# ericdegroot/gr-ldpc_ece535a

Measured on AMD Instinct MI355X. Metric: decoded info Mbit/s @ 50 BP iters, batch=4096; achieved HBM GB/s vs peak, higher is better.
Workload: dtype f64

## Files before the change

### gr-ldpc_ece535a_amd/csrc/ldpc_capi_create.hip

```cpp
#include <stdio.h>

#include <exception>

#include "ldpc_ctx.hpp"
#include "ldpc_layout.hpp"
#include "ldpc_qc.hpp"

using namespace ldpc::capi;
using ldpc::ColRec;
using ldpc::EdgeColRec;
using ldpc::EdgeRowRec;
using ldpc::kNone;

namespace ldpc {
namespace capi {

int set_err(ldpc_ctx *ctx, int code, const std::string &msg) {
  if (!ctx) return set_create_error(code, msg);
  ctx->err = msg;
  return code;
}

int hip_err(ldpc_ctx *ctx, hipError_t e, const char *what) {
  return set_err(ctx, LDPC_EDEVICE, std::string(what) + ": " + hipGetErrorString(e));
// ... 52 lines not shown
        row_edges[j].push_back(e);
        col_edges[i].push_back(e);
      }
  code.E = (int)erow.size();
  code.dc_max = 0;
  code.dv_max = 0;
  for (auto &r : row_edges) code.dc_max = std::max(code.dc_max, (int)r.size());
  code.dc_min = code.dc_max;
  for (auto &r : row_edges) code.dc_min = std::min(code.dc_min, (int)r.size());
  for (auto &c : col_edges) code.dv_max = std::max(code.dv_max, (int)c.size());
  if (code.E == 0) return set_err(ctx, LDPC_EINVAL, "H has no ones");
  if (N > ldpc::kNMax || M > ldpc::kMMax || code.E > 64 * ldpc::kSlotsMax ||
      code.dc_max > ldpc::kDcMax || code.dv_max > ldpc::kDvMax) {
    char buf[256];
    snprintf(buf, sizeof buf,
             "code shape outside the small-code kernel (M=%d N=%d E=%d dc_max=%d dv_max=%d; "
             "limits M,N<=%d E<=%d dc<=%d dv<=%d)",
             M, N, code.E, code.dc_max, code.dv_max, ldpc::kNMax, 64 * ldpc::kSlotsMax,
             ldpc::kDcMax, ldpc::kDvMax);
    return set_err(ctx, LDPC_EUNSUPPORTED, buf);
  }
  ctx->slots = (code.E + 63) / 64;
  ctx->nw = N <= 64 ? 1 : 4;
  ctx->rs = (M + 63) / 64;
  const int slots = ctx->slots, nw = ctx->nw;
  code.K = N - M;
  code.KB = (code.K + 7) / 8;

  const ldpc::KernelShape shape = ldpc::kernel_shape(nw, slots, code.dc_max, code.dv_max);
  const ldpc::EdgeLayout lay = ldpc::plan_layout(M, N, erow, ecol, slots, nw, shape.dcn, shape.dvn,
                                                 shape.cols, search);
  const std::vector<int> &cell = lay.slot, &pos = lay.pos;
  if (cell_out) *cell_out = cell;
  int *model = ctx->small.layout_model;
  model[0] = lay.searched ? 1 : 0;
  model[1] = lay.model_cc;
  model[2] = lay.model_ec;
  model[3] = lay.plain_cc;
  model[4] = lay.plain_ec;
  uint64_t *dpos = ctx->small.dpos;
  dpos[0] = dpos[1] = 0;
  for (int g = 0; g < 2 * slots; ++g) dpos[g / 8] |= (uint64_t)(lay.dpos[g] & 31) << (8 * (g % 8));

  erecs.assign((size_t)64 * slots, EdgeRowRec{});
  crecs.assign((size_t)64 * slots, EdgeColRec{});
  for (auto &r : erecs) {
    std::fill(std::begin(r.rn), std::end(r.rn), kNone);
    r.col = kNone;
  }
  for (auto &r : crecs) {
    std::fill(std::begin(r.cn), std::end(r.cn), kNone);
    r.col = kNone;
  }
  for (int e = 0; e < code.E; ++e) {
    EdgeRowRec &er = erecs[cell[e]];
    EdgeColRec &ec = crecs[cell[e]];
    er.col = ec.col = (uint16_t)pos[ecol[e]];
    int k = 0;
    for (int n : row_edges[erow[e]])
      if (n != e) er.rn[k++] = (uint16_t)cell[n];
    k = 0;
    for (int n : col_edges[ecol[e]])
      if (n != e) ec.cn[k++] = (uint16_t)cell[n];
  }
  cols.assign((size_t)64 * nw, ColRec{});
  for (auto &c : cols) {
    std::fill(std::begin(c.e), std::end(c.e), kNone);
    std::fill(std::begin(c.r), std::end(c.r), kNone);
  }
  lane_col.assign((size_t)64 * nw, kNone);
  col_lane.assign((size_t)N, 0);
  for (int i = 0; i < N; ++i) {
    lane_col[pos[i]] = (uint16_t)i;
    col_lane[i] = (uint8_t)pos[i];
    for (size_t k = 0; k < col_edges[i].size(); ++k) {
      cols[pos[i]].e[k] = (uint16_t)cell[col_edges[i][k]];
      cols[pos[i]].r[k] = (uint16_t)erow[col_edges[i][k]];
    }
  }
  rowmask.assign((size_t)M * nw, 0);
  for (int j = 0; j < M; ++j)
    for (int i = 0; i < N; ++i)
      if (H[(size_t)j * N + i]) rowmask[(size_t)j * nw + pos[i] / 64] |= 1ull << (pos[i] % 64);
  return LDPC_OK;
}

int build_graph(ldpc_ctx *ctx, std::vector<int32_t> &cp, std::vector<int32_t> &ce,
                std::vector<int32_t> &cr) {
  ldpc_ctx::Code &code = ctx->code;
  const int M = code.M, N = code.N;
  code.E = code.rp[M];
  if (code.E == 0) return set_err(ctx, LDPC_EINVAL, "H has no ones");
  cp.assign((size_t)N + 1, 0);
  for (int e = 0; e < code.E; ++e) cp[code.ci[e] + 1]++;
  code.dc_max = 0;
  code.dv_max = 0;
  for (int i = 0; i < N; ++i) code.dv_max = std::max(code.dv_max, cp[i + 1]);
  for (int j = 0; j < M; ++j) code.dc_max = std::max(code.dc_max, code.rp[j + 1] - code.rp[j]);
  for (int i = 0; i < N; ++i) cp[i + 1] += cp[i];
  ce.assign((size_t)code.E, 0);
  cr.assign((size_t)code.E, 0);
  std::vector<int32_t> fill(cp.begin(), cp.end() - 1);
  for (int j = 0; j < M; ++j)
    for (int32_t e = code.rp[j]; e < code.rp[j + 1]; ++e) {
      const int32_t k = fill[code.ci[e]]++;
      ce[k] = e;
      cr[k] = j;
    }
  if (code.dc_max > ldpc::kGraphDcMax || code.dv_max > ldpc::kGraphDvMax) {
    char buf[160];
    snprintf(buf, sizeof buf,
             "code degrees outside the large-code kernels (dc_max=%d dv_max=%d; limits %d, %d)",
             code.dc_max, code.dv_max, ldpc::kGraphDcMax, ldpc::kGraphDvMax);
    return set_err(ctx, LDPC_EUNSUPPORTED, buf);
  }
  code.K = N - M;
  code.KB = (code.K + 7) / 8;
  ctx->graph.on = true;
  return LDPC_OK;
}

int check_onchip(ldpc_ctx *ctx) {
  const ldpc_ctx::Code &code = ctx->code;
  for (int method = 0; method < 2; ++method)
    for (int prec = 0; prec < 4; ++prec) {
      ldpc::OnchipLayout L;
      if (ldpc::onchip_plan(code.M, code.N, code.E, code.dc_max, code.dv_max, method, prec, L))
        continue;
      char buf[256];
      if (L.frame > ldpc::kOnchipLdsLimit)
        snprintf(buf, sizeof buf,
                 "the code does not fit the on-chip kernels: a frame needs %d bytes of LDS "
                 "(method %d, precision %d), the limit is %d (M=%d N=%d E=%d)",
                 L.frame, method, prec, ldpc::kOnchipLdsLimit, code.M, code.N, code.E);
      else
        snprintf(buf, sizeof buf,
                 "the code does not fit the on-chip kernels: M, N, E must be <= %d (M=%d N=%d "
                 "E=%d; a frame needs %d bytes of LDS, the limit is %d)",
                 ldpc::kOnchipIndexMax, code.M, code.N, code.E, L.frame, ldpc::kOnchipLdsLimit);
      return set_err(ctx, LDPC_EUNSUPPORTED, buf);
    }
  return LDPC_OK;
}

ldpc_ctx *finish_create(ldpc_ctx *ctx, int flags, int device) {
  std::vector<EdgeRowRec> erecs;
  std::vector<EdgeColRec> crecs;
  std::vector<ColRec> cols;
  std::vector<uint64_t> rowmask;
  std::vector<uint16_t> lane_col;
  std::vector<uint8_t> col_lane;
  std::vector<int32_t> cp, ce, cr;
  ldpc_ctx::Code &code = ctx->code;
  ldpc_ctx::Graph &graph = ctx->graph;
  const auto refuse = [&](const std::string &msg) -> ldpc_ctx * {
    set_err(nullptr, LDPC_EINVAL, msg);
    delete ctx;
    return nullptr;
  };
  const bool onchip = (flags & LDPC_FLAG_ONCHIP) != 0;
  if (onchip && (flags & LDPC_FLAG_GRAPH))
    return refuse("LDPC_FLAG_ONCHIP and LDPC_FLAG_GRAPH exclude each other");
  ldpc::OnchipTables oct;
  int rc = LDPC_EUNSUPPORTED;
  if (!(flags & (LDPC_FLAG_GRAPH | LDPC_FLAG_ONCHIP)) && !code.H.empty())
    rc = build_tables(ctx, erecs, crecs, cols, rowmask, lane_col, col_lane,
// ... 351 lines not shown
```

### gr-ldpc_ece535a_amd/csrc/ldpc_device.hpp

```cpp
#pragma once

#include <hip/hip_runtime.h>

#include <float.h>
#include <math.h>

#include "ldpc_exact.hpp"
#include "ldpc_math.hpp"

namespace ldpc {

template <int PREC>
struct Math;

__device__ const ex::ExTab kExTab = ex::make_ex_tab();
__device__ const fm::LogTabEntry kLogTab[1 << fm::kLogTabBits] = {LDPC_LOGTAB_ENTRIES};

template <>
struct Math<0> {
  typedef double Real;
  typedef ex::ExTab Tab;
  static constexpr int kTabN = 1;
  static __device__ __forceinline__ const Tab *tab_src() { return &kExTab; }
  template <int n>
  static __device__ __forceinline__ void tanh_half_n(const double (&m)[n], double (&z)[n],
                                                     const Tab *tab) {
    ex::tanh_half_n<n>(m, z, tab);
  }
  template <int n>
  static __device__ __forceinline__ void check_msg_n(const double (&T)[n], const Tab *tab,
                                                     double (&E)[n]) {
    ex::log_ratio_n<n>(T, tab, E);
  }
  static __device__ __forceinline__ double tanh_half(double m, const Tab *tab) {
    const double v[1] = {m};
    double z[1];
    ex::tanh_half_n<1>(v, z, tab);
    return z[0];
  }
  static __device__ __forceinline__ double check_msg(double T, const Tab *tab) {
    const double v[1] = {T};
    double e[1];
    ex::log_ratio_n<1>(v, tab, e);
    return e[0];
  }
  static __device__ __forceinline__ double abs_(double x) { return ::fabs(x); }
  static __device__ __forceinline__ double max_() { return DBL_MAX; }
};
template <>
struct Math<2> : Math<0> {
  template <int n>
  static __device__ __forceinline__ void tanh_half_n(const double (&m)[n], double (&z)[n],
                                                     const Tab *tab) {
#pragma unroll
    for (int i = 0; i < n; ++i) z[i] = Math<0>::tanh_half(m[i], tab);
  }
  template <int n>
  static __device__ __forceinline__ void check_msg_n(const double (&T)[n], const Tab *tab,
                                                     double (&E)[n]) {
#pragma unroll
    for (int i = 0; i < n; ++i) E[i] = Math<0>::check_msg(T[i], tab);
  }
};
template <>
struct Math<3> {
  typedef double Real;
  typedef fm::LogTabEntry Tab;
  static constexpr int kTabN = 1 << fm::kLogTabBits;
  static __device__ __forceinline__ const Tab *tab_src() { return kLogTab; }
#ifdef LDPC_TANH_SINGLE_RANGE
  static __device__ __forceinline__ double tanh_half(double m, const Tab * = nullptr) {
    return fm::tanh_half_fast(m);
  }
#else
  static __device__ __forceinline__ double tanh_half(double m, const Tab * = nullptr) {
    return fm::tanh_half_acc(m);
  }
#endif
  static __device__ __forceinline__ double check_msg(double T, const Tab *tab) {
    return fm::log_ratio_tab(T, tab);
  }
  template <int n>
  static __device__ __forceinline__ void tanh_half_n(const double (&m)[n], double (&z)[n],
                                                     const Tab *) {
#pragma unroll
    for (int i = 0; i < n; ++i) z[i] = tanh_half(m[i]);
  }
  template <int n>
  static __device__ __forceinline__ void check_msg_n(const double (&T)[n], const Tab *tab,
                                                     double (&E)[n]) {
#pragma unroll
    for (int i = 0; i < n; ++i) E[i] = check_msg(T[i], tab);
  }
  static __device__ __forceinline__ double abs_(double x) { return ::fabs(x); }
  static __device__ __forceinline__ double max_() { return DBL_MAX; }
};
template <>
struct Math<1> {
  typedef float Real;
  typedef float Tab;
  static constexpr int kTabN = 0;
  static __device__ __forceinline__ const Tab *tab_src() { return nullptr; }
  static __device__ __forceinline__ float tanh_half(float m, const Tab * = nullptr) {
    return ::tanhf(m / 2.0f);
  }
  static __device__ __forceinline__ float check_msg(float T, const Tab *) {
    return ::logf((1.0f + T) / (1.0f - T));
  }
  template <int n>
  static __device__ __forceinline__ void tanh_half_n(const float (&m)[n], float (&z)[n],
                                                     const Tab *) {
#pragma unroll
    for (int i = 0; i < n; ++i) z[i] = tanh_half(m[i]);
  }
  template <int n>
  static __device__ __forceinline__ void check_msg_n(const float (&T)[n], const Tab *tab,
                                                     float (&E)[n]) {
#pragma unroll
    for (int i = 0; i < n; ++i) E[i] = check_msg(T[i], tab);
  }
  static __device__ __forceinline__ float abs_(float x) { return ::fabsf(x); }
  static __device__ __forceinline__ float max_() { return FLT_MAX; }
};

template <int n>
__device__ __forceinline__ void log_ratio_n_packed(const double (&T)[n],
                                                   const ex::ExTab *tab, double (&E)[n],
                                                   double *scratch, int lane, uint32_t zero_at) {
  double q[n];
  const bool any_special = ex::ratio_n<n>(T, q);
  uint32_t pos[n];
  bool near[n], packed[n];
  uint32_t base = 0;
#pragma unroll
  for (int i = 0; i < n; ++i) {
    E[i] = ex::log_main(q[i], tab->log);
    near[i] = ex::log_is_near1(q[i]);
    const bool unit = q[i] == 1.0;
    packed[i] = near[i] && !unit;
    const uint64_t m = LDPC_EX_LANES(near[i]) & LDPC_EX_LANES(!unit);
    pos[i] = unit ? zero_at
                  : base + __builtin_amdgcn_mbcnt_hi((uint32_t)(m >> 32),
                                                     __builtin_amdgcn_mbcnt_lo((uint32_t)m, 0u));
    base += (uint32_t)__builtin_popcountll(m);
  }
  asm volatile("" ::: "memory");
  if (base != 0) {
#pragma unroll
    for (int i = 0; i < n; ++i)
      if (packed[i]) scratch[pos[i]] = q[i];
    asm volatile("" ::: "memory");
    for (uint32_t p = 0; p < base; p += 64) {
      const uint32_t idx = p + (uint32_t)lane;
      if (idx < base) scratch[idx] = ex::log_near1(scratch[idx]);
    }
    asm volatile("" ::: "memory");
  }
#pragma unroll
  for (int i = 0; i < n; ++i)
    if (near[i]) E[i] = scratch[pos[i]];
  asm volatile("" ::: "memory");
  if (any_special) {
    LDPC_EX_COLD();
    ex::ratio_fix_n<n>(T, E);
  }
}

template <int PREC>
struct TabLds {
  typedef typename Math<PREC>::Tab Tab;
  static constexpr int kN = Math<PREC>::kTabN > 0 ? Math<PREC>::kTabN : 1;
};
template <int PREC>
__device__ __forceinline__ void stage_tab(typename Math<PREC>::Tab *lds) {
  if constexpr (Math<PREC>::kTabN > 0) {
    typedef typename Math<PREC>::Tab Tab;
    static_assert(sizeof(Tab) % 4 == 0, "tables are copied in 32-bit words");
    constexpr int words = (int)(sizeof(Tab) / 4) * Math<PREC>::kTabN;
    const uint32_t *src = reinterpret_cast<const uint32_t *>(Math<PREC>::tab_src());
    uint32_t *dst = reinterpret_cast<uint32_t *>(lds);
    for (int i = threadIdx.x; i < words; i += blockDim.x) dst[i] = src[i];
    __syncthreads();
  }
}

template <typename Real>
__device__ __forceinline__ int sgn(Real v) {
  return (v > Real(0)) - (v < Real(0));
}

}
```

### gr-ldpc_ece535a_amd/csrc/ldpc_exact.hpp

```cpp
#pragma once

#include <stdint.h>
#include <string.h>

#include "ldpc_glibc_log.hpp"

#ifndef LDPC_HD
#if defined(__HIPCC__)
#define LDPC_HD __host__ __device__ __forceinline__
#else
#define LDPC_HD inline
#endif
#endif

#if defined(__HIP_DEVICE_COMPILE__)
#define LDPC_EX_ANY(c) (__builtin_amdgcn_ballot_w64(c) != 0)
#define LDPC_EX_LANES(c) __builtin_amdgcn_ballot_w64(c)
#define LDPC_EX_SCALAR_COPY(x) asm("" : "+s"(x))
#define LDPC_EX_COLD() asm volatile(";ldpc_cold")
#else
#define LDPC_EX_ANY(c) (c)
#define LDPC_EX_LANES(c) ((uint64_t)(c))
#define LDPC_EX_SCALAR_COPY(x) ((void)0)
#define LDPC_EX_COLD() ((void)0)
#endif

namespace ldpc {
namespace ex {

LDPC_HD uint64_t bits(double x) {
  uint64_t u;
  memcpy(&u, &x, 8);
  return u;
}
LDPC_HD double dbl(uint64_t u) {
  double x;
  memcpy(&x, &u, 8);
  return x;
}
LDPC_HD uint32_t hiw(double x) { return (uint32_t)(bits(x) >> 32); }
LDPC_HD double from_hi(uint32_t h) { return dbl((uint64_t)h << 32); }
LDPC_HD double fma_(double a, double b, double c) { return __builtin_fma(a, b, c); }
LDPC_HD double sel(bool c, double a, double b) { return c ? a : b; }

#if !defined(__HIP_DEVICE_COMPILE__)
inline int g_rcp_perturb_ulps = 0;
#endif

LDPC_HD double rcp_seed(double p) {
#if defined(__HIP_DEVICE_COMPILE__)
  return __builtin_amdgcn_rcp(p);
#else
  return dbl(bits(1.0 / p) + (int64_t)g_rcp_perturb_ulps);
#endif
}

LDPC_HD double div_core(double a, double b, double yk) {
  const double q0 = a * yk;
  const double r = fma_(-b, q0, a);
  double q1 = fma_(r, yk, q0);
  const double r1 = fma_(-b, q1, a);
  const bool flag = fma_(r1, yk, q1) != q1;
  if (LDPC_EX_ANY(flag)) {
    LDPC_EX_COLD();
    const bool down = ((hiw(r1) ^ hiw(b) ^ hiw(q1)) & 0x80000000u) != 0;
    const uint32_t e = down ? (uint32_t)((bits(q1) - 1) >> 32) : hiw(q1);
    const double h = from_hi((e & 0x7ff00000u) - (53u << 20));
    const bool wrong = fma_(-__builtin_fabs(b), h, __builtin_fabs(r1)) > 0.0;
    q1 = wrong ? dbl(bits(q1) + (down ? ~0ull : 1ull)) : q1;
  }
  return q1;
}

template <int n>
LDPC_HD void div_recips(const double (&b)[n], double (&yk)[n]) {
  double p[n];
  p[0] = b[0];
#pragma unroll
  for (int i = 1; i < n; ++i) p[i] = p[i - 1] * b[i];
  double y = rcp_seed(p[n - 1]);
  y = fma_(fma_(-p[n - 1], y, 1.0 + 0x1p-40), y, y);
#pragma unroll
  for (int i = n - 1; i > 0; --i) {
    yk[i] = y * p[i - 1];
    y = y * b[i];
  }
  yk[0] = y;
}

template <int n>
LDPC_HD void div_n(const double (&a)[n], const double (&b)[n], double (&q)[n]) {
  double yk[n];
  div_recips<n>(b, yk);
#pragma unroll
  for (int i = n - 1; i >= 0; --i) q[i] = div_core(a[i], b[i], yk[i]);
}

struct RedEntry {
  double khi, klo;
};
struct TailEntry {
  double a, b;
};
constexpr int kTailLo = -3, kTailN = 68;
constexpr double kLn2Hi = 6.93147180369123816490e-01;
constexpr double kLn2Lo = 1.90821492927058770002e-10;
constexpr RedEntry red_entry(int k) { return RedEntry{(double)k * kLn2Hi, (double)k * kLn2Lo}; }
constexpr TailEntry tail_entry(int k) {
  return TailEntry{(k == 0 || k == -1) ? 0.0
                   : (k >= 2 && k <= 19) ? 1.0 - 1.0 / (double)(1ull << k)
                                         : 1.0,
                   k == -1 ? -0.5 : (k >= 0 && k <= 56) ? -0.0 : -1.0};
}
struct ExTab {
  GlLogEntry log[1 << kGlTabBits];
  RedEntry red[kTailN];
  TailEntry tail[kTailN];
};
constexpr ExTab make_ex_tab() {
  ExTab t{{LDPC_GLIBC_LOG_TAB}, {}, {}};
  for (int k = kTailLo; k < kTailLo + kTailN; ++k) {
    t.red[k - kTailLo] = red_entry(k);
    t.tail[k - kTailLo] = tail_entry(k);
  }
  return t;
}

template <int n>
LDPC_HD void expm1_n(const double (&u)[n], const uint32_t (&hx)[n], double (&t)[n], int (&k)[n],
                     const ExTab *tab, bool mid_possible = true) {
  constexpr double invln2 = 1.44269504088896338700e+00;
  constexpr double Q1 = -3.33333333333331316428e-02;
  constexpr double Q2 = 1.58730158725481460165e-03;
  constexpr double Q3 = -7.93650757867487942473e-05;
  constexpr double Q4 = 4.00821782732936239552e-06;
  constexpr double Q5 = -2.01099218183624371326e-07;
  double x[n], c[n], hxs[n], num[n], den[n], q[n];
  bool edge = false;
#pragma unroll
  for (int i = 0; i < n; ++i) {
    k[i] = (int)__builtin_copysign(invln2 * __builtin_fabs(u[i]) + 0.5, u[i]);
    edge |= hx[i] == 0x3fd62e42u;
  }
  if (LDPC_EX_ANY(edge)) {
    LDPC_EX_COLD();
#pragma unroll
    for (int i = 0; i < n; ++i) k[i] = hx[i] > 0x3fd62e42u ? k[i] : 0;
  }
#pragma unroll
  for (int i = 0; i < n; ++i) {
    const RedEntry re = tab->red[k[i] - kTailLo];
    const double hi = u[i] - re.khi;
    const double lo = re.klo;
    x[i] = hi - lo;
    c[i] = (hi - x[i]) - lo;
    const double hfx = 0.5 * x[i];
    hxs[i] = x[i] * hfx;
    const double h = hxs[i];
    const double R1 = 1.0 + h * Q1, h2 = h * h;
    const double R2 = Q2 + h * Q3, h4 = h2 * h2;
    const double R3 = Q4 + h * Q5;
    const double r1 = R1 + h2 * R2 + h4 * R3;
    const double tt = 3.0 - r1 * hfx;
    num[i] = r1 - tt;
    den[i] = 6.0 - x[i] * tt;
  }
  div_n<n>(num, den, q);
  bool any_mid = false;
  double ep[n];
#pragma unroll
  for (int i = 0; i < n; ++i) {
    const double e = hxs[i] * q[i];
    ep[i] = (x[i] * (e - c[i]) - c[i]) - hxs[i];
    const double d = ep[i] - x[i];
    const int kk = k[i];
    const TailEntry te = tab->tail[kk - kTailLo];
    t[i] = __builtin_ldexp(te.a - d, kk) + te.b;
  }
  if (mid_possible) {
#pragma unroll
    for (int i = 0; i < n; ++i) any_mid |= (uint32_t)(k[i] - 20) <= 36u;
  }
  if (mid_possible && LDPC_EX_ANY(any_mid)) {
    LDPC_EX_COLD();
#pragma unroll
    for (int i = 0; i < n; ++i) {
      const int kk = k[i];
      const int km = kk < 20 ? 20 : (kk > 56 ? 56 : kk);
      const double tm = from_hi((uint32_t)(0x3ff - km) << 20);
      const double y = (x[i] - (ep[i] + tm)) + 1.0;
      const double v = y * from_hi((uint32_t)(0x3ff + km) << 20);
      t[i] = (uint32_t)(kk - 20) <= 36u ? v : t[i];
    }
  }
}

template <int n>
LDPC_HD void expm1_n(const double (&u)[n], double (&t)[n], const ExTab *tab,
                     bool mid_possible = true) {
  uint32_t hx[n];
#pragma unroll
  for (int i = 0; i < n; ++i) hx[i] = hiw(u[i]) & 0x7fffffffu;
  int k[n];
  expm1_n<n>(u, hx, t, k, tab, mid_possible);
}

template <int n>
LDPC_HD void tanh_half_n(const double (&m)[n], double (&z)[n], const ExTab *tab) {
  static_assert(n <= 8, "the tanh divisors (up to 2^63 each) share one prefix product");
  double u[n], t[n], num[n], den[n], q[n];
  uint32_t hm[n];
  uint64_t special = 0;
#pragma unroll
  for (int i = 0; i < n; ++i) {
    hm[i] = hiw(m[i]);
    const uint32_t im = hm[i] & 0x7fffffffu;
    u[i] = dbl(((uint64_t)(im | ((im - 0x40000000u) & 0x80000000u)) << 32) | (uint32_t)bits(m[i]));
    special |= LDPC_EX_LANES(im - 0x3c900000u >= 0x402b0000u - 0x3c900000u) &
               LDPC_EX_LANES(m[i] != 0.0);
  }
  const bool any_special = special != 0;
  uint64_t special_again = special;
  LDPC_EX_SCALAR_COPY(special_again);
  if (any_special) {
    LDPC_EX_COLD();
#pragma unroll
    for (int i = 0; i < n; ++i) {
      const uint32_t im = hm[i] & 0x7fffffffu;
      const double ac = __builtin_fmin(__builtin_fmax(__builtin_fabs(m[i]), 0x1p-54), 43.0);
      u[i] = dbl(bits(ac) ^ ((uint64_t)((im - 0x40000000u) & 0x80000000u) << 32));
    }
  }
  uint32_t hx[n];
#pragma unroll
  for (int i = 0; i < n; ++i) hx[i] = hm[i] & 0x7fffffffu;
  int k[n];
  expm1_n<n>(u, hx, t, k, tab, any_special);
#pragma unroll
  for (int i = 0; i < n; ++i) {
    const bool big = k[i] > 0;
    num[i] = big ? 2.0 : -t[i];
    den[i] = t[i] + 2.0;
  }
  div_n<n>(num, den, q);
#pragma unroll
  for (int i = 0; i < n; ++i) {
    const bool big = k[i] > 0;
    const double r = q[i] + from_hi(big ? 0xbff00000u : 0u);
    const uint32_t zh = (hiw(r) & 0x7fffffffu) | (hm[i] & 0x80000000u);
    z[i] = dbl(((uint64_t)zh << 32) | (uint32_t)bits(r));
  }
  if (special_again != 0) {
    LDPC_EX_COLD();
#pragma unroll
    for (int i = 0; i < n; ++i) {
      const double x = m[i] * 0.5;
      const uint32_t ix = hiw(x) & 0x7fffffffu;
      z[i] = ix < 0x3c800000u ? x * (1.0 + x) : (x != x ? x + x : z[i]);
    }
  }
}

LDPC_HD double log_main(double q, const GlLogEntry *tab) {
  const uint64_t ix = bits(q);
  const uint32_t th = (uint32_t)(ix >> 32) - 0x3fe60000u;
  const int k = (int32_t)th >> 20;
  const double z = __builtin_ldexp(q, -k);
  static_assert(sizeof(GlLogEntry) == 16, "16-byte log table entries");
  const uint32_t off = (th >> (20 - kGlTabBits - 4)) & (((1u << kGlTabBits) - 1) << 4);
  const GlLogEntry e = *reinterpret_cast<const GlLogEntry *>(reinterpret_cast<const char *>(tab) + off);
  const double r = fma_(z, e.invc, -1.0);
  const double kd = (double)k;
  const double w = fma_(kd, kGlLn2hi, e.logc);
  const double hi = w + r;
  const double lo = fma_(kd, kGlLn2lo, (w - hi) + r);
  const double r2 = r * r;
  const double r3 = r * r2;
  const double p = fma_(fma_(r, kGlA[4], kGlA[3]), r2, fma_(r, kGlA[2], kGlA[1]));
  return fma_(r3, p, fma_(r2, kGlA[0], lo)) + hi;
}

LDPC_HD double log_near1(double q) {
  const double r = q - 1.0;
  const double r2 = r * r;
  const double r3 = r * r2;
  const double P1 = fma_(r2, kGlB[3], fma_(r, kGlB[2], kGlB[1]));
  const double P2 = fma_(r2, kGlB[6], fma_(r, kGlB[5], kGlB[4]));
  const double P3 = fma_(r3, kGlB[10], fma_(r2, kGlB[9], fma_(r, kGlB[8], kGlB[7])));
  const double poly = fma_(fma_(P3, r3, P2), r3, P1);
  const double W = fma_(r, 0x1p27, r);
  const double rhi = fma_(-0x1p27, r, W);
  const double rlo = r - rhi;
  const double rh2 = rhi * rhi;
  const double hi = fma_(rh2, kGlB[0], r);
  const double lo = fma_(rh2, kGlB[0], r - hi);
  const double lo2 = fma_(kGlB[0] * rlo, r + rhi, lo);
  return fma_(poly, r3, lo2) + hi;
}

LDPC_HD bool log_is_near1(double q) { return hiw(q) - 0x3fee0000u < 0x3ff10900u - 0x3fee0000u; }

LDPC_HD double log_q(double q, const GlLogEntry *tab) {
  double y = log_main(q, tab);
  const bool near = log_is_near1(q);
  if (LDPC_EX_ANY(near)) {
    LDPC_EX_COLD();
    y = near ? log_near1(q) : y;
  }
  return y;
}

inline double log_main_bits(uint64_t ix, const GlLogEntry *tab) {
  const uint32_t th = (uint32_t)(ix >> 32) - 0x3fe60000u;
  const uint32_t i = (th >> (20 - kGlTabBits)) & ((1u << kGlTabBits) - 1);
  const int k = (int32_t)th >> 20;
  const uint64_t iz = ((uint64_t)((uint32_t)(ix >> 32) - (th & 0xfff00000u)) << 32) | (uint32_t)ix;
  const GlLogEntry e = tab[i];
  const double z = dbl(iz);
  const double r = fma_(z, e.invc, -1.0);
  const double kd = (double)k;
  const double w = fma_(kd, kGlLn2hi, e.logc);
  const double hi = w + r;
  const double lo = fma_(kd, kGlLn2lo, (w - hi) + r);
  const double r2 = r * r;
  const double r3 = r * r2;
  const double p = fma_(fma_(r, kGlA[4], kGlA[3]), r2, fma_(r, kGlA[2], kGlA[1]));
  return fma_(r3, p, fma_(r2, kGlA[0], lo)) + hi;
}

inline double log_glibc(double x, const GlLogEntry *tab) {
  uint64_t ix = bits(x);
  if (log_is_near1(x)) return ix == bits(1.0) ? 0.0 : log_near1(x);
  const uint32_t top = (uint32_t)(ix >> 48);
  if (top - 0x0010u >= 0x7ff0u - 0x0010u) {
    if ((ix << 1) == 0) return -__builtin_inf();
    if (ix == bits(__builtin_inf())) return x;
    if ((top & 0x8000u) || (top & 0x7ff0u) == 0x7ff0u) return (x - x) / 0.0;
    ix = bits(x * 0x1p52) - (52ull << 52);
    return log_main_bits(ix, tab);
  }
  return log_main(dbl(ix), tab);
}

template <int n>
LDPC_HD bool ratio_n(const double (&T)[n], double (&q)[n]) {
  static_assert(n <= 16, "the divisors (>= 2^-53 each) share one prefix product");
  double num[n], den[n];
  bool special = false;
#pragma unroll
  for (int i = 0; i < n; ++i) {
    num[i] = 1.0 + T[i];
    den[i] = 1.0 - T[i];
    special |= LDPC_EX_ANY(!(__builtin_fabs(T[i]) < 1.0));
  }
  if (special) {
    LDPC_EX_COLD();
#pragma unroll
    for (int i = 0; i < n; ++i) den[i] = __builtin_fmax(den[i], 0x1p-60);
  }
  div_n<n>(num, den, q);
  return special;
}

template <int n>
LDPC_HD void ratio_fix_n(const double (&T)[n], double (&E)[n]) {
#pragma unroll
  for (int i = 0; i < n; ++i)
    E[i] = __builtin_fabs(T[i]) < 1.0
               ? E[i]
               : (T[i] != T[i] ? T[i] + T[i] : __builtin_copysign(__builtin_inf(), T[i]));
}

template <int n>
LDPC_HD void log_ratio_n(const double (&T)[n], const ExTab *tab, double (&E)[n]) {
  double q[n];
  const bool any_special = ratio_n<n>(T, q);
#pragma unroll
  for (int i = 0; i < n; ++i) E[i] = log_q(q[i], tab->log);
  if (any_special) {
    LDPC_EX_COLD();
    ratio_fix_n<n>(T, E);
  }
// ... 5 lines not shown
```

### gr-ldpc_ece535a_amd/csrc/ldpc_frame.hpp

```cpp
#pragma once

#include <hip/hip_runtime.h>

#include <float.h>
#include <math.h>

#include <algorithm>

#include "ldpc_device.hpp"
#include "ldpc_kernels.hpp"
#include "ldpc_layout.hpp"
#include "ldpc_wgframe.hpp"

namespace ldpc {

__device__ __forceinline__ void wave_lds_sync() {
#ifdef LDPC_LDS_FENCE
  __builtin_amdgcn_fence(__ATOMIC_RELEASE, "wavefront");
  __builtin_amdgcn_wave_barrier();
  __builtin_amdgcn_fence(__ATOMIC_ACQUIRE, "wavefront");
#else
  __builtin_amdgcn_wave_barrier();
  asm volatile("" ::: "memory");
#endif
// ... 52 lines not shown
    const uint32_t ad = base / size + (id == kNone ? dummy : id);
    p[k >> 1] = (p[k >> 1] & ~(0xffffu << ((k & 1) * 16))) | (ad << ((k & 1) * 16));
  }
}
template <typename Real, int W>
__device__ __forceinline__ uint32_t lds_at(const uint32_t (&p)[W], int k) {
  return (uint32_t)field(p, k) * (uint32_t)sizeof(Real);
}

__host__ __device__ constexpr size_t align16(size_t x) { return (x + 15) & ~size_t(15); }

template <int METHOD, int S, int NW, int DVN>
__host__ __device__ constexpr bool cols_kernel() {
  return cols_form(METHOD, S, NW, DVN);
}

template <typename Real, int METHOD, int S, int NW, int DVN>
struct Layout {
  static constexpr SliceLayout L{S, NW, cols_kernel<METHOD, S, NW, DVN>()};
  static constexpr size_t per_wave = align16((size_t)L.end * sizeof(Real));
  static constexpr size_t total = (size_t)kWavesPerBlock * per_wave;
};

__device__ __forceinline__ uint32_t dpos_of(const CodeView &code, int g) {
  const uint64_t w = g < 8 ? code.dpos[0] : code.dpos[1];
  return (uint32_t)(w >> (8 * (g & 7))) & 31u;
}

template <int S, int NW>
struct WaveTables {
  uint32_t rn[S][4];
  uint32_t cn[S][2];
  uint32_t ce[NW][2];
  uint32_t cr[NW][2];
  uint64_t rowmask[NW][NW];
};

struct FrameResult {
  int weight;
  uint32_t byte;
  int used;
};
template <int PREC, int METHOD, int S, int NW, int DCN = kDcMax - 1, int DVN = kDvMax,
          bool FIN = false, typename Real = typename Math<PREC>::Real, bool OUT = true,
          bool FAIR = true>
__device__ __forceinline__ FrameResult decode_frame(const CodeView &code, const DecodeArgs &a,
                                             const int64_t b, WaveTables<S, NW> &wt,
                                             Real *tb, Real *eb, Real *rb, Real *sb,
                                             const int lane,
                                             const typename Math<PREC>::Tab *logtab,
                                             const float (&xin)[NW], const int (&colq)[NW],
                                             const uint32_t (&ppos)[2]) {
  const int M = code.M, N = code.N;
  constexpr int kDummy = 64 * S;
  constexpr SliceLayout L = Layout<Real, METHOD, S, NW, DVN>::L;
  Real post[NW];
#pragma unroll
  for (int q = 0; q < NW; ++q) {
    const int c = lane + 64 * q;
    Real r = -(Real)xin[q];
    asm volatile("" : "+v"(r));
    rb[c] = r;
    post[q] = (Real)xin[q];
  }

  uint64_t hard[NW];
#pragma unroll
  for (int q = 0; q < NW; ++q) hard[q] = 0;
  int weight = 0, used = 0;
  uint64_t col_ok[NW], row_ok[NW];
#pragma unroll
  for (int q = 0; q < NW; ++q) {
    col_ok[q] = __ballot(lane + 64 * q < N);
    row_ok[q] = __ballot(lane + 64 * q < M);
  }

  auto syndrome = [&]() {
    int w = 0;
#pragma unroll
    for (int q = 0; q < NW; ++q) {
      int odd = 0;
#pragma unroll
      for (int k = 0; k < NW; ++k) odd ^= __popcll(wt.rowmask[q][k] & hard[k]);
      w += __popcll(__builtin_amdgcn_ballot_w64((odd & 1) != 0) & row_ok[q]);
    }
    return w;
  };

  constexpr bool kCols = cols_kernel<METHOD, S, NW, DVN>();
  if constexpr (kCols) {
    const uint32_t eb_dummy = lds_addr(eb + kDummy + (lane & 31));
    constexpr uint32_t kTbEb = (uint32_t)(L.eb - L.tb) * sizeof(Real);
    if (lane < 32) {
      tb[kDummy + lane] = Real(1);
      eb[kDummy + lane] = Real(0);
    }
    uint32_t ra[S][DCN], ea[NW][DVN], ta[NW][DVN];
#pragma unroll
    for (int s = 0; s < S; ++s)
#pragma unroll
      for (int k = 0; k < DCN; ++k) ra[s][k] = lds_at<Real>(wt.rn[s], k);
    Real *nr = sb + 64 * NW;
#pragma unroll
    for (int q = 0; q < NW; ++q)
#pragma unroll
      for (int k = 0; k < DVN; ++k) {
        const uint32_t e = lds_at<Real>(wt.ce[q], k);
        ta[q][k] = e == eb_dummy ? lds_addr(tb + L.jk + lane + 64 * q) : e - kTbEb;
        ea[q][k] = (FIN && e == eb_dummy) ? lds_addr(nr + lane + 64 * q) : e;
      }
    Real rc[NW];
    bool open = FIN && PREC == 3 && LDPC_TANH_SPLIT > 0;
#pragma unroll
    for (int q = 0; q < NW; ++q) {
      rc[q] = rb[lane + 64 * q];
      if constexpr (FIN) nr[lane + 64 * q] = -rc[q];
      const Real t0 = Math<PREC>::tanh_half(rc[q], logtab);
      open = open && __builtin_amdgcn_ballot_w64(!(__builtin_fabs((double)rc[q]) <=
                                                    LDPC_TANH_SPLIT)) == 0;
#pragma unroll
      for (int k = 0; k < DVN; ++k) lds_st<Real>(ta[q][k], t0);
    }
#ifdef LDPC_PATH_STATS
    bool st_same = false;
    double st_prev[NW][DVN];
#pragma unroll
    for (int q = 0; q < NW; ++q)
#pragma unroll
      for (int k = 0; k < DVN; ++k) st_prev[q][k] = __builtin_nan("");
#endif
    const uint32_t fair = FAIR ? a.fair_cycles : 0u;
    uint64_t t_prev = fair ? __builtin_amdgcn_s_memtime() : 0;
    for (int h = 0; h < a.max_iters; ++h) {
      const uint64_t now = fair ? __builtin_amdgcn_s_memtime() : 0;
      wave_lds_sync();
      Real nb[S][DCN];
#pragma unroll
      for (int s = 0; s < S; ++s)
#pragma unroll
        for (int k = 0; k < DCN; ++k) nb[s][k] = lds_ld<Real>(ra[s][k]);
#pragma unroll
      for (int s = 0; s < S; ++s)
#pragma unroll
        for (int k = 0; k < DCN; ++k) asm volatile("" ::"v"(nb[s][k]));
      Real Ts[S];
#pragma unroll
      for (int s = 0; s < S; ++s) {
        Real T = Real(1);
#pragma unroll
        for (int k = 0; k < DCN; ++k) T = T * nb[s][k];
        Ts[s] = T;
      }
      if constexpr (PREC != 3) {
        Real Es[S];
        if constexpr (PREC == 0)
          log_ratio_n_packed<S>(Ts, logtab, Es, tb, lane, (uint32_t)(L.ebd - L.tb));
        else
          Math<PREC>::template check_msg_n<S>(Ts, logtab, Es);
#ifdef LDPC_PATH_STATS
        if constexpr (PREC == 0) {
          bool some = false, all = true, same = true;
#pragma unroll
          for (int s = 0; s < S; ++s) {
            const double T = (double)Ts[s];
            const bool sat = !(__builtin_fabs(T) < 1.0);
            some |= sat;
            all &= sat || T == 0.0;
            same &= __builtin_bit_cast(uint64_t, (double)Es[s]) ==
                    __builtin_bit_cast(uint64_t, (double)eb[lane + 64 * s]);
          }
          const bool s1 = __ballot(some) != 0, a1 = __ballot(!all) == 0, e1 = __ballot(!same) == 0;
          st_same = e1;
          int nbase = 0, nunit = 0;
#pragma unroll
          for (int s = 0; s < S; ++s) {
            const double T = (double)Ts[s], q = (1.0 + T) / (1.0 - T);
            const bool near = ex::log_is_near1(q);
            nbase += __popcll(__ballot(near));
            nunit += __popcll(__ballot(near && q == 1.0));
          }
          if (lane == 0) {
            atomicAdd(&g_path_stats[8], (unsigned long long)nbase);
            if (nbase > 64) atomicAdd(&g_path_stats[9], 1ull);
            atomicAdd(&g_path_stats[10], (unsigned long long)nunit);
            if (nbase - nunit > 64) atomicAdd(&g_path_stats[11], 1ull);
            atomicAdd(&g_path_stats[0], 1ull);
            if (s1) atomicAdd(&g_path_stats[1], 1ull);
            if (a1) atomicAdd(&g_path_stats[2], 1ull);
            if (e1) atomicAdd(&g_path_stats[5], 1ull);
          }
        }
#endif
#pragma unroll
        for (int s = 0; s < S; ++s) eb[lane + 64 * s] = Es[s];
      } else if constexpr (FIN && LDPC_TANH_SPLIT > 0) {
        if (open) {
#ifdef LDPC_NO_BATCH_DIV
#pragma unroll
          for (int s = 0; s < S; ++s) eb[lane + 64 * s] = fm::log_ratio_tab_open(Ts[s], logtab);
#else
          if (code.dc_min >= 2) {
            Real Es[S];
            fm::log_ratio_tab_open_n<S>(Ts, logtab, Es);
#pragma unroll
            for (int s = 0; s < S; ++s) eb[lane + 64 * s] = Es[s];
          } else {
#pragma unroll
            for (int s = 0; s < S; ++s) eb[lane + 64 * s] = fm::log_ratio_tab_open(Ts[s], logtab);
          }
#endif
        } else {
#pragma unroll
          for (int s = 0; s < S; ++s) eb[lane + 64 * s] = Math<PREC>::check_msg(Ts[s], logtab);
        }
      } else {
#pragma unroll
        for (int s = 0; s < S; ++s) eb[lane + 64 * s] = Math<PREC>::check_msg(Ts[s], logtab);
      }
      if (fair) {
        const uint32_t d = (uint32_t)(now - t_prev);
        t_prev = now;
        if (d > fair)
          __builtin_amdgcn_s_setprio(3);
        else
          __builtin_amdgcn_s_setprio(0);
      }
      wave_lds_sync();
      Real tv[NW][DVN];
#pragma unroll
      for (int q = 0; q < NW; ++q) {
        Real ev[DVN];
#pragma unroll
        for (int k = 0; k < DVN; ++k) ev[k] = lds_ld<Real>(ea[q][k]);
#pragma unroll
        for (int k = 0; k < DVN; ++k) tv[q][k] = ev[k] + rc[q];
        Real acc = Real(0);
        if constexpr (FIN) {
          acc = tv[q][0];
#pragma unroll
          for (int k = 1; k < DVN; ++k) acc = acc + tv[q][k];
        } else {
#pragma unroll
          for (int k = 0; k < DVN; ++k) acc = ea[q][k] != eb_dummy ? acc + tv[q][k] : acc;
        }
        post[q] = acc;
        hard[q] = __builtin_amdgcn_ballot_w64(acc <= Real(0)) & col_ok[q];
      }
      Real mv[NW][DVN];
#pragma unroll
      for (int q = 0; q < NW; ++q)
#pragma unroll
        for (int k = 0; k < DVN; ++k) {
          Real m = Real(0);
          bool first = true;
#pragma unroll
          for (int k2 = 0; k2 < DVN; ++k2) {
            if (k2 == k) continue;
            if constexpr (FIN)
              m = first ? tv[q][k2] : m + tv[q][k2];
            else
              m = ea[q][k2] != eb_dummy ? m + tv[q][k2] : m;
            first = false;
          }
          mv[q][k] = m;
        }
#ifdef LDPC_PATH_STATS
      if constexpr (PREC == 0) {
        bool some = false, all = true, same = true, big = false;
#pragma unroll
        for (int q = 0; q < NW; ++q)
#pragma unroll
          for (int k = 0; k < DVN; ++k) {
            const double m = (double)mv[q][k], am = __builtin_fabs(m);
            some |= !(am >= 0x1p-54 && am < 13.5) && am != 0.0;
            big |= am >= 13.5;
            all &= !(am < 38.2);
            same &= __builtin_bit_cast(uint64_t, m) == __builtin_bit_cast(uint64_t, st_prev[q][k]);
            st_prev[q][k] = m;
          }
        const bool s1 = __ballot(some) != 0, a1 = __ballot(!all) == 0, e1 = __ballot(!same) == 0;
        const bool b1 = __ballot(big) != 0;
        if (lane == 0) {
          if (s1) atomicAdd(&g_path_stats[3], 1ull);
          if (b1) atomicAdd(&g_path_stats[7], 1ull);
          if (a1) atomicAdd(&g_path_stats[4], 1ull);
          if (e1 && st_same) atomicAdd(&g_path_stats[6], 1ull);
        }
      }
#endif
      weight = syndrome();
      used = h + 1;
      if (h + 1 == a.max_iters) break;
      if ((h + 1) % a.et_period == 0 && weight == 0) break;
      if constexpr (PREC != 3) {
#pragma unroll
        for (int q = 0; q < NW; ++q) {
          Real th[DVN];
          Math<PREC>::template tanh_half_n<DVN>(mv[q], th, logtab);
#pragma unroll
          for (int k = 0; k < DVN; ++k) lds_st<Real>(ta[q][k], th[k]);
        }
      } else if constexpr (LDPC_TANH_SPLIT > 0) {
        bool wide = false;
#pragma unroll
        for (int q = 0; q < NW; ++q)
#pragma unroll
          for (int k = 0; k < DVN; ++k) wide |= !(__builtin_fabs(mv[q][k]) <= LDPC_TANH_SPLIT);
        if (__builtin_amdgcn_ballot_w64(wide) == 0) {
#pragma unroll
          for (int q = 0; q < NW; ++q) {
#ifdef LDPC_NO_BATCH_DIV
#pragma unroll
            for (int k = 0; k < DVN; ++k) lds_st<Real>(ta[q][k], fm::tanh_half_small(mv[q][k]));
#else
            Real th[DVN];
            fm::tanh_half_small_n<DVN>(mv[q], th);
#pragma unroll
            for (int k = 0; k < DVN; ++k) lds_st<Real>(ta[q][k], th[k]);
#endif
          }
          open = FIN;
        } else {
#pragma unroll
          for (int q = 0; q < NW; ++q)
#pragma unroll
            for (int k = 0; k < DVN; ++k) lds_st<Real>(ta[q][k], Math<PREC>::tanh_half(mv[q][k], logtab));
          open = false;
        }
      } else {
#pragma unroll
        for (int q = 0; q < NW; ++q)
#pragma unroll
          for (int k = 0; k < DVN; ++k) lds_st<Real>(ta[q][k], Math<PREC>::tanh_half(mv[q][k], logtab));
      }
    }
  } else if constexpr (METHOD == 1 || METHOD == 0) {
    const uint32_t eb_dummy = lds_addr(eb + kDummy + (lane & 31));
    if (lane < 32) {
      tb[kDummy + lane] = METHOD == 1 ? Real(1) : Math<PREC>::max_();
      eb[kDummy + lane] = Real(0);
    }
    uint32_t col[S], ra[S][DCN], ca[S][DVN - 1], ea[NW][DVN];
#pragma unroll
    for (int s = 0; s < S; ++s) {
      col[s] = lds_at<Real>(wt.rn[s], 7);
#pragma unroll
      for (int k = 0; k < DCN; ++k) ra[s][k] = lds_at<Real>(wt.rn[s], k);
#pragma unroll
      for (int k = 0; k < DVN - 1; ++k) ca[s][k] = lds_at<Real>(wt.cn[s], k);
    }
#pragma unroll
    for (int q = 0; q < NW; ++q)
#pragma unroll
      for (int k = 0; k < DVN; ++k) ea[q][k] = lds_at<Real>(wt.ce[q], k);
    if constexpr (METHOD == 1 && FIN) {
      Real *nr = sb + 64 * NW;
#pragma unroll
      for (int s = 0; s < S; ++s)
#pragma unroll
        for (int k = 0; k < DVN - 1; ++k)
          ca[s][k] = ca[s][k] == eb_dummy ? lds_addr(nr + lane + 64 * s) : ca[s][k];
#pragma unroll
      for (int q = 0; q < NW; ++q)
#pragma unroll
        for (int k = 0; k < DVN; ++k)
          ea[q][k] = ea[q][k] == eb_dummy ? lds_addr(nr + 64 * S + lane + 64 * q) : ea[q][k];
    }
    constexpr uint32_t kSb = 64 * NW * sizeof(Real);
    wave_lds_sync();
    Real msg[S];
    Real lr[S];
#pragma unroll
    for (int s = 0; s < S; ++s) {
      msg[s] = lds_ld<Real>(col[s]);
      lr[s] = Real(0);
    }
    if constexpr (METHOD == 1 && FIN) {
      Real *nr = sb + 64 * NW;
#pragma unroll
      for (int s = 0; s < S; ++s) nr[lane + 64 * s] = -msg[s];
#pragma unroll
// ... 489 lines not shown
```

Before: 1498.

## Trim exact-precision tanh/log paths using precomputed zero-lane masks and lean kernels

```diff
diff --git a/gr-ldpc_ece535a_amd/csrc/ldpc_capi_create.hip b/gr-ldpc_ece535a_amd/csrc/ldpc_capi_create.hip
--- a/gr-ldpc_ece535a_amd/csrc/ldpc_capi_create.hip
+++ b/gr-ldpc_ece535a_amd/csrc/ldpc_capi_create.hip
@@ -158,6 +158,13 @@
   for (int j = 0; j < M; ++j)
     for (int i = 0; i < N; ++i)
       if (H[(size_t)j * N + i]) rowmask[(size_t)j * nw + pos[i] / 64] |= 1ull << (pos[i] % 64);
+  rowmask.resize((size_t)M * nw + (size_t)nw * ldpc::kDvMax, 0);
+  for (int p = 0; p < 64 * nw; ++p)
+    for (int k = 0; k < ldpc::kDvMax; ++k) {
+      bool alone = true;
+      for (int k2 = 0; k2 < ldpc::kDvMax; ++k2) alone = alone && (k2 == k || cols[p].e[k2] == kNone);
+      if (alone) rowmask[(size_t)M * nw + (size_t)(p / 64) * ldpc::kDvMax + k] |= 1ull << (p % 64);
+    }
   return LDPC_OK;
 }
 
diff --git a/gr-ldpc_ece535a_amd/csrc/ldpc_device.hpp b/gr-ldpc_ece535a_amd/csrc/ldpc_device.hpp
--- a/gr-ldpc_ece535a_amd/csrc/ldpc_device.hpp
+++ b/gr-ldpc_ece535a_amd/csrc/ldpc_device.hpp
@@ -26,6 +26,11 @@
   static __device__ __forceinline__ void tanh_half_n(const double (&m)[n], double (&z)[n],
                                                      const Tab *tab) {
     ex::tanh_half_n<n>(m, z, tab);
+  }
+  template <int n>
+  static __device__ __forceinline__ void tanh_half_n(const double (&m)[n], double (&z)[n],
+                                                     const Tab *tab, const uint64_t (&zero)[n]) {
+    ex::tanh_half_n<n>(m, z, tab, zero);
   }
   template <int n>
   static __device__ __forceinline__ void check_msg_n(const double (&T)[n], const Tab *tab,
@@ -123,7 +128,7 @@
   static __device__ __forceinline__ float max_() { return FLT_MAX; }
 };
 
-template <int n>
+template <int n, bool LEAN = false>
 __device__ __forceinline__ void log_ratio_n_packed(const double (&T)[n],
                                                    const ex::ExTab *tab, double (&E)[n],
                                                    double *scratch, int lane, uint32_t zero_at) {
@@ -150,9 +155,20 @@
     for (int i = 0; i < n; ++i)
       if (packed[i]) scratch[pos[i]] = q[i];
     asm volatile("" ::: "memory");
-    for (uint32_t p = 0; p < base; p += 64) {
-      const uint32_t idx = p + (uint32_t)lane;
-      if (idx < base) scratch[idx] = ex::log_near1(scratch[idx]);
+    if constexpr (LEAN) {
+      if ((uint32_t)lane < base) scratch[lane] = ex::log_near1_lean(scratch[lane]);
+      if (base > 64) {
+        LDPC_EX_COLD();
+        for (uint32_t p = 64; p < base; p += 64) {
+          const uint32_t idx = p + (uint32_t)lane;
+          if (idx < base) scratch[idx] = ex::log_near1_lean(scratch[idx]);
+        }
+      }
+    } else {
+      for (uint32_t p = 0; p < base; p += 64) {
+        const uint32_t idx = p + (uint32_t)lane;
+        if (idx < base) scratch[idx] = ex::log_near1(scratch[idx]);
+      }
     }
     asm volatile("" ::: "memory");
   }
diff --git a/gr-ldpc_ece535a_amd/csrc/ldpc_exact.hpp b/gr-ldpc_ece535a_amd/csrc/ldpc_exact.hpp
--- a/gr-ldpc_ece535a_amd/csrc/ldpc_exact.hpp
+++ b/gr-ldpc_ece535a_amd/csrc/ldpc_exact.hpp
@@ -42,6 +42,15 @@
 LDPC_HD double from_hi(uint32_t h) { return dbl((uint64_t)h << 32); }
 LDPC_HD double fma_(double a, double b, double c) { return __builtin_fma(a, b, c); }
 LDPC_HD double sel(bool c, double a, double b) { return c ? a : b; }
+LDPC_HD double fma3_(double s, double a, double c) {
+#if defined(__HIP_DEVICE_COMPILE__)
+  double d;
+  asm("v_fma_f64 %0, %1, %2, %3" : "=v"(d) : "s"(s), "v"(a), "v"(c));
+  return d;
+#else
+  return __builtin_fma(s, a, c);
+#endif
+}
 
 #if !defined(__HIP_DEVICE_COMPILE__)
 inline int g_rcp_perturb_ulps = 0;
@@ -126,7 +135,7 @@
   return t;
 }
 
-template <int n>
+template <int n, bool LEAN = false>
 LDPC_HD void expm1_n(const double (&u)[n], const uint32_t (&hx)[n], double (&t)[n], int (&k)[n],
                      const ExTab *tab, bool mid_possible = true) {
   constexpr double invln2 = 1.44269504088896338700e+00;
@@ -147,9 +156,22 @@
 #pragma unroll
     for (int i = 0; i < n; ++i) k[i] = hx[i] > 0x3fd62e42u ? k[i] : 0;
   }
-#pragma unroll
-  for (int i = 0; i < n; ++i) {
-    const RedEntry re = tab->red[k[i] - kTailLo];
+  static_assert(sizeof(RedEntry) == 16 && sizeof(TailEntry) == 16, "16-byte per-k entries");
+  int koff[n];
+#pragma unroll
+  for (int i = 0; i < n; ++i) {
+    RedEntry re;
+    if constexpr (LEAN) {
+      koff[i] = k[i] * 16;
+#if defined(__HIP_DEVICE_COMPILE__)
+      asm("" : "+v"(koff[i]));
+#endif
+      re = *reinterpret_cast<const RedEntry *>(reinterpret_cast<const char *>(tab->red - kTailLo) +
+                                               koff[i]);
+    } else {
+      koff[i] = 0;
+      re = tab->red[k[i] - kTailLo];
+    }
     const double hi = u[i] - re.khi;
     const double lo = re.klo;
     x[i] = hi - lo;
@@ -174,7 +196,12 @@
     ep[i] = (x[i] * (e - c[i]) - c[i]) - hxs[i];
     const double d = ep[i] - x[i];
     const int kk = k[i];
-    const TailEntry te = tab->tail[kk - kTailLo];
+    TailEntry te;
+    if constexpr (LEAN)
+      te = *reinterpret_cast<const TailEntry *>(reinterpret_cast<const char *>(tab->tail - kTailLo) +
+                                                koff[i]);
+    else
+      te = tab->tail[kk - kTailLo];
     t[i] = __builtin_ldexp(te.a - d, kk) + te.b;
   }
   if (mid_possible) {
@@ -205,10 +232,11 @@
   expm1_n<n>(u, hx, t, k, tab, mid_possible);
 }
 
-template <int n>
-LDPC_HD void tanh_half_n(const double (&m)[n], double (&z)[n], const ExTab *tab) {
+template <int n, bool MASKED, bool LEAN>
+LDPC_HD void tanh_half_impl(const double (&m)[n], double (&z)[n], const ExTab *tab,
+                            const uint64_t *zero) {
   static_assert(n <= 8, "the tanh divisors (up to 2^63 each) share one prefix product");
-  double u[n], t[n], num[n], den[n], q[n];
+  double u[n], t[n], num[n], nneg[n], den[n], q[n];
   uint32_t hm[n];
   uint64_t special = 0;
 #pragma unroll
@@ -216,8 +244,11 @@
     hm[i] = hiw(m[i]);
     const uint32_t im = hm[i] & 0x7fffffffu;
     u[i] = dbl(((uint64_t)(im | ((im - 0x40000000u) & 0x80000000u)) << 32) | (uint32_t)bits(m[i]));
-    special |= LDPC_EX_LANES(im - 0x3c900000u >= 0x402b0000u - 0x3c900000u) &
-               LDPC_EX_LANES(m[i] != 0.0);
+    if constexpr (MASKED)
+      special |= LDPC_EX_LANES(im - 0x3c900000u >= 0x402b0000u - 0x3c900000u) & ~zero[i];
+    else
+      special |= LDPC_EX_LANES(im - 0x3c900000u >= 0x402b0000u - 0x3c900000u) &
+                 LDPC_EX_LANES(m[i] != 0.0);
   }
   const bool any_special = special != 0;
   uint64_t special_again = special;
@@ -235,18 +266,23 @@
 #pragma unroll
   for (int i = 0; i < n; ++i) hx[i] = hm[i] & 0x7fffffffu;
   int k[n];
-  expm1_n<n>(u, hx, t, k, tab, any_special);
+  expm1_n<n, LEAN>(u, hx, t, k, tab, any_special);
 #pragma unroll
   for (int i = 0; i < n; ++i) {
     const bool big = k[i] > 0;
-    num[i] = big ? 2.0 : -t[i];
+    nneg[i] = big ? -2.0 : t[i];
+    num[i] = -nneg[i];
     den[i] = t[i] + 2.0;
   }
   div_n<n>(num, den, q);
 #pragma unroll
   for (int i = 0; i < n; ++i) {
     const bool big = k[i] > 0;
-    const double r = q[i] + from_hi(big ? 0xbff00000u : 0u);
+    double w = from_hi(big ? 0xbff00000u : 0u);
+    if constexpr (LEAN) {
+      w = dbl(((uint64_t)(big ? 0xbff00000u : 0u) << 32) | (uint32_t)bits(nneg[i]));
+    }
+    const double r = q[i] + w;
     const uint32_t zh = (hiw(r) & 0x7fffffffu) | (hm[i] & 0x80000000u);
     z[i] = dbl(((uint64_t)zh << 32) | (uint32_t)bits(r));
   }
@@ -259,6 +295,16 @@
       z[i] = ix < 0x3c800000u ? x * (1.0 + x) : (x != x ? x + x : z[i]);
     }
   }
+}
+
+template <int n>
+LDPC_HD void tanh_half_n(const double (&m)[n], double (&z)[n], const ExTab *tab) {
+  tanh_half_impl<n, false, false>(m, z, tab, nullptr);
+}
+template <int n>
+LDPC_HD void tanh_half_n(const double (&m)[n], double (&z)[n], const ExTab *tab,
+                         const uint64_t (&zero)[n]) {
+  tanh_half_impl<n, true, true>(m, z, tab, zero);
 }
 
 LDPC_HD double log_main(double q, const GlLogEntry *tab) {
@@ -298,6 +344,24 @@
   return fma_(poly, r3, lo2) + hi;
 }
 
+LDPC_HD double log_near1_lean(double q) {
+  const double r = q - 1.0;
+  const double r2 = r * r;
+  const double r3 = r * r2;
+  const double P1 = fma_(r2, kGlB[3], fma3_(kGlB[2], r, kGlB[1]));
+  const double P2 = fma_(r2, kGlB[6], fma3_(kGlB[5], r, kGlB[4]));
+  const double P3 = fma_(r3, kGlB[10], fma_(r2, kGlB[9], fma3_(kGlB[8], r, kGlB[7])));
+  const double poly = fma_(fma_(P3, r3, P2), r3, P1);
+  const double W = fma3_(0x1p27, r, r);
+  const double rhi = fma_(-0x1p27, r, W);
+  const double rlo = r - rhi;
+  const double rh2 = rhi * rhi;
+  const double hi = fma_(rh2, kGlB[0], r);
+  const double lo = fma_(rh2, kGlB[0], r - hi);
+  const double lo2 = fma_(kGlB[0] * rlo, r + rhi, lo);
+  return fma_(poly, r3, lo2) + hi;
+}
+
 LDPC_HD bool log_is_near1(double q) { return hiw(q) - 0x3fee0000u < 0x3ff10900u - 0x3fee0000u; }
 
 LDPC_HD double log_q(double q, const GlLogEntry *tab) {
diff --git a/gr-ldpc_ece535a_amd/csrc/ldpc_frame.hpp b/gr-ldpc_ece535a_amd/csrc/ldpc_frame.hpp
--- a/gr-ldpc_ece535a_amd/csrc/ldpc_frame.hpp
+++ b/gr-ldpc_ece535a_amd/csrc/ldpc_frame.hpp
@@ -158,7 +158,10 @@
       int odd = 0;
 #pragma unroll
       for (int k = 0; k < NW; ++k) odd ^= __popcll(wt.rowmask[q][k] & hard[k]);
-      w += __popcll(__builtin_amdgcn_ballot_w64((odd & 1) != 0) & row_ok[q]);
+      if constexpr (cols_kernel<METHOD, S, NW, DVN>() && FIN && PREC == 0)
+        w += __popcll(__builtin_amdgcn_ballot_w64((odd & 1) != 0));
+      else
+        w += __popcll(__builtin_amdgcn_ballot_w64((odd & 1) != 0) & row_ok[q]);
     }
     return w;
   };
@@ -185,6 +188,26 @@
         ta[q][k] = e == eb_dummy ? lds_addr(tb + L.jk + lane + 64 * q) : e - kTbEb;
         ea[q][k] = (FIN && e == eb_dummy) ? lds_addr(nr + lane + 64 * q) : e;
       }
+    constexpr bool kZeroLanes = FIN && PREC == 0;
+    uint64_t zl[NW][DVN];
+    if constexpr (kZeroLanes) {
+#pragma unroll
+      for (int q = 0; q < NW; ++q) {
+        uint64_t w[DVN];
+#pragma unroll
+        for (int k = 0; k < DVN; ++k) {
+          const uint64_t v = code.rowmask[M * NW + q * kDvMax + k];
+          w[k] = ((uint64_t)(uint32_t)__builtin_amdgcn_readfirstlane((int)(v >> 32)) << 32) |
+                 (uint32_t)__builtin_amdgcn_readfirstlane((int)(uint32_t)v);
+        }
+        zl[q][0] = w[0];
+        uint64_t rest = ~0ull;
+#pragma unroll
+        for (int k = 1; k < DVN; ++k) rest &= w[k];
+#pragma unroll
+        for (int k = 1; k < DVN; ++k) zl[q][k] = rest;
+      }
+    }
     Real rc[NW];
     bool open = FIN && PREC == 3 && LDPC_TANH_SPLIT > 0;
 #pragma unroll
@@ -230,7 +253,7 @@
       if constexpr (PREC != 3) {
         Real Es[S];
         if constexpr (PREC == 0)
-          log_ratio_n_packed<S>(Ts, logtab, Es, tb, lane, (uint32_t)(L.ebd - L.tb));
+          log_ratio_n_packed<S, true>(Ts, logtab, Es, tb, lane, (uint32_t)(L.ebd - L.tb));
         else
           Math<PREC>::template check_msg_n<S>(Ts, logtab, Es);
 #ifdef LDPC_PATH_STATS
@@ -372,7 +395,10 @@
 #pragma unroll
         for (int q = 0; q < NW; ++q) {
           Real th[DVN];
-          Math<PREC>::template tanh_half_n<DVN>(mv[q], th, logtab);
+          if constexpr (kZeroLanes)
+            Math<PREC>::template tanh_half_n<DVN>(mv[q], th, logtab, zl[q]);
+          else
+            Math<PREC>::template tanh_half_n<DVN>(mv[q], th, logtab);
 #pragma unroll
           for (int k = 0; k < DVN; ++k) lds_st<Real>(ta[q][k], th[k]);
         }
```

Result: faster. 1526, median of 6 (+1.9%).
